# staple/spark-agd

Measured on NVIDIA H100. Metric: AGD examples/sec (rows x applySmooth passes / s), logistic 10M x 1024 dense fp32, higher is better.
Workload: dtype f64

## Files before the change

### spark-agd_b200/csrc/k1_tc.cu

```cuda
#include <cuda.h>
#include <cuda_bf16.h>
#include <cuda_runtime.h>
#include <stdint.h>

#include "agd_common.cuh"
#include "k1_device.cuh"

namespace agd {

namespace {

constexpr int kKR = 16;
constexpr int kRegsConsumer = 64, kRegsAux = 56, kRegsMma = 168;
constexpr int kBlockBytes = kKR * 128;
constexpr int kBBytes = 1024;
constexpr int kScaleOff = 768;

__device__ __forceinline__ uint32_t smem_u32(const void *p) { return (uint32_t)__cvta_generic_to_shared(p); }
__device__ __forceinline__ void mbar_init(uint32_t bar, uint32_t count) {
  asm volatile("mbarrier.init.shared::cta.b64 [%0], %1;" ::"r"(bar), "r"(count));
}
__device__ __forceinline__ void mbar_expect_tx(uint32_t bar, uint32_t bytes) {
  asm volatile("mbarrier.arrive.expect_tx.shared::cta.b64 _, [%0], %1;" ::"r"(bar), "r"(bytes) : "memory");
}
__device__ __forceinline__ void mbar_arrive(uint32_t bar) {
  asm volatile("mbarrier.arrive.shared::cta.b64 _, [%0];" ::"r"(bar) : "memory");
}
__device__ __forceinline__ void mbar_wait(uint32_t bar, uint32_t parity) {
  asm volatile(
      "{\n\t.reg .pred p;\n\t"
      "WAIT_LOOP:\n\t"
      "mbarrier.try_wait.parity.shared::cta.b64 p, [%0], %1;\n\t"
      "@p bra WAIT_DONE;\n\t"
      "bra WAIT_LOOP;\n\t"
      "WAIT_DONE:\n\t}" ::"r"(bar),
      "r"(parity)
      : "memory");
}
__device__ __forceinline__ void named_arrive(int id, int count) {
  asm volatile("bar.arrive %0, %1;" ::"r"(id), "r"(count) : "memory");
}
__device__ __forceinline__ void named_sync(int id, int count) {
  asm volatile("bar.sync %0, %1;" ::"r"(id), "r"(count) : "memory");
}
__device__ __forceinline__ void tma_bulk_g2s(uint32_t dst, const void *src, uint32_t bytes, uint32_t bar) {
  asm volatile("cp.async.bulk.shared::cluster.global.mbarrier::complete_tx::bytes [%0], [%1], %2, [%3];" ::"r"(dst),
               "l"(src), "r"(bytes), "r"(bar)
               : "memory");
}
__device__ __forceinline__ void tma_tile_2d(uint32_t dst, const CUtensorMap *map, int c0, int c1, uint32_t bar) {
  asm volatile("cp.async.bulk.tensor.2d.shared::cluster.global.mbarrier::complete_tx::bytes [%0], [%1, {%2, %3}], [%4];" ::"r"(dst),
               "l"(map), "r"(c0), "r"(c1), "r"(bar)
               : "memory");
}
__device__ __forceinline__ void tma_tile_3d(uint32_t dst, const CUtensorMap *map, int c0, int c1, int c2, uint32_t bar) {
  asm volatile("cp.async.bulk.tensor.3d.shared::cluster.global.mbarrier::complete_tx::bytes [%0], [%1, {%2, %3, %4}], [%5];" ::"r"(dst),
               "l"(map), "r"(c0), "r"(c1), "r"(c2), "r"(bar)
               : "memory");
}
__device__ __forceinline__ uint64_t gmma_desc(uint32_t addr, uint32_t lbo, uint32_t sbo, uint64_t layout) {
  return (uint64_t)((addr & 0x3FFFF) >> 4) | ((uint64_t)(lbo >> 4) << 16) | ((uint64_t)(sbo >> 4) << 32) | (layout << 62);
}
__device__ __forceinline__ void wgmma_fence() { asm volatile("wgmma.fence.sync.aligned;" ::: "memory"); }
__device__ __forceinline__ void wgmma_commit() { asm volatile("wgmma.commit_group.sync.aligned;" ::: "memory"); }
template <int N>
__device__ __forceinline__ void wgmma_wait() { asm volatile("wgmma.wait_group.sync.aligned %0;" ::"n"(N) : "memory"); }
template <int N>
__device__ __forceinline__ void wgmma_bf16(float (&d)[N / 2], uint64_t adesc, uint64_t bdesc);
template <>
__device__ __forceinline__ void wgmma_bf16<16>(float (&d)[8], uint64_t adesc, uint64_t bdesc) {
  asm volatile("{ .reg .pred p; setp.ne.b32 p, 0, 0;\n\t"
               "wgmma.mma_async.sync.aligned.m64n16k16.f32.bf16.bf16 {%0,%1,%2,%3,%4,%5,%6,%7}, %8, %9, p, 1, 1, 1, 0; }"
               : "+f"(d[0]), "+f"(d[1]), "+f"(d[2]), "+f"(d[3]), "+f"(d[4]), "+f"(d[5]), "+f"(d[6]), "+f"(d[7])
               : "l"(adesc), "l"(bdesc)
               : "memory");
}
template <>
__device__ __forceinline__ void wgmma_bf16<24>(float (&d)[12], uint64_t adesc, uint64_t bdesc) {
  asm volatile("{ .reg .pred p; setp.ne.b32 p, 0, 0;\n\t"
               "wgmma.mma_async.sync.aligned.m64n24k16.f32.bf16.bf16 {%0,%1,%2,%3,%4,%5,%6,%7,%8,%9,%10,%11}, %12, %13, p, 1, 1, 1, 0; }"
               : "+f"(d[0]), "+f"(d[1]), "+f"(d[2]), "+f"(d[3]), "+f"(d[4]), "+f"(d[5]), "+f"(d[6]), "+f"(d[7]),
                 "+f"(d[8]), "+f"(d[9]), "+f"(d[10]), "+f"(d[11])
               : "l"(adesc), "l"(bdesc)
               : "memory");
}

template <int N, bool TWO>
__device__ __forceinline__ void mma_accumulate(const float (&e)[2][N / 2], int hb, int hs, const double (&sc)[2], double &g,
                                               double *g2) {
  float v[6];
#pragma unroll
  for (int t = 0; t < (TWO ? 6 : 3); ++t) {
    const int i = t == 0 ? 0 : t == 1 ? 1 : t == 2 ? 4 : t == 3 ? 5 : t == 4 ? 8 : 9;
    const float x0 = hs ? e[0][i + 2] : e[0][i], x1 = hs ? e[1][i + 2] : e[1][i];
    v[t] = hb ? x1 : x0;
  }
  g += (((double)v[0] + (double)v[1]) + (double)v[2]) * sc[0];
  if (TWO) *g2 += (((double)v[3] + (double)v[4]) + (double)v[5]) * sc[1];
}
__device__ __forceinline__ double pow2i(int k) { return __longlong_as_double((long long)(k + 1023) << 52); }
__device__ __forceinline__ void mma_release(uint32_t empty_bar, int lane) {
  __syncwarp();
  if (lane == 0) mbar_arrive(empty_bar);
}

struct TcLayout {
  uint32_t ring_off, w_off, b2_off, partial_off, bars_off, g2_off, total;
};
__host__ __device__ inline TcLayout tc_layout(int ring_groups, int group_bytes, int d, bool two_gradient) {
  TcLayout L;
  L.ring_off = 0;
  L.w_off = (uint32_t)ring_groups * group_bytes;
  L.b2_off = L.w_off + (uint32_t)d * 8;
  L.partial_off = L.b2_off + 2 * kBBytes;
  L.bars_off = L.partial_off + 2 * kKR * 16 * 8;
  L.g2_off = L.bars_off + (2 * (uint32_t)ring_groups + 8) * 8;
  L.total = L.g2_off + (two_gradient ? (uint32_t)d * 8 : 0u);
  return L;
}

struct TcArgs {
  const double *labels;
  const double *w;
  const double *w2;
  double *slabs;
  long long rows;
  int d, kind, slab_stride;
  unsigned long long sample_seed, sample_thresh;
  long long row_base;
  const RowFilter *filt;
  const uint32_t *view_bits;
  int gb;
  int ngt;
  int ring_groups;
  int one_copy;
  int diag;
};

__host__ __device__ constexpr int tc_consumers(int rpt) { return rpt == 4 ? 256 : 512; }
__device__ __forceinline__ unsigned long long ffma2(unsigned long long a, unsigned long long b, unsigned long long c) {
  const float x = __fmaf_rn(__uint_as_float((uint32_t)a), __uint_as_float((uint32_t)b), __uint_as_float((uint32_t)c));
  const float y = __fmaf_rn(__uint_as_float((uint32_t)(a >> 32)), __uint_as_float((uint32_t)(b >> 32)),
                            __uint_as_float((uint32_t)(c >> 32)));
  return ((unsigned long long)__float_as_uint(y) << 32) | __float_as_uint(x);
}
__device__ __forceinline__ unsigned long long pack2(uint32_t lo, uint32_t hi) {
  unsigned long long d;
  asm("mov.b64 %0, {%1, %2};" : "=l"(d) : "r"(lo), "r"(hi));
  return d;
}

template <int RPT, bool F32, int DUAL, bool VIEW, bool BIAS>
__global__ void __launch_bounds__(tc_consumers(RPT) + 256, 1)
k1_tc_kernel(const __grid_constant__ CUtensorMap tmap, const __grid_constant__ CUtensorMap tmap3, const TcArgs a,
             const long long ntiles) {
  constexpr int kConsumers = tc_consumers(RPT);
  constexpr int kThreads = kConsumers + 256;
  constexpr int kN = DUAL == 2 ? 24 : 16;
  constexpr int kCW = kConsumers / 32;
  constexpr bool kRepartition = RPT != 4;
  extern __shared__ __align__(1024) unsigned char smem[];
  const int group_bytes = a.gb * kBlockBytes;
  const TcLayout L = tc_layout(a.ring_groups, group_bytes, a.d, DUAL == 2);
  double *w_s = reinterpret_cast<double *>(smem + L.w_off);
  unsigned char *b2 = smem + L.b2_off;
  double *partial = reinterpret_cast<double *>(smem + L.partial_off);
  const uint32_t bars = smem_u32(smem + L.bars_off);
  const int RG = a.ring_groups;
  const uint32_t wbar = bars + 16u * RG, b2_full = wbar + 8, b2_empty = b2_full + 16;
  const int tid = threadIdx.x, warp = tid >> 5, lane = tid & 31;
  const long long my_tiles = (ntiles - blockIdx.x + gridDim.x - 1) / gridDim.x;
  const int npairs = a.d / 128;
  double *slab = a.slabs + (size_t)blockIdx.x * a.slab_stride;

  if (tid == 0) {
    for (int g = 0; g < RG; ++g) {
      mbar_init(bars + 8u * g, 1);
      mbar_init(bars + 8u * (RG + g), 4);
    }
    mbar_init(wbar, 1);
    mbar_init(b2_full, 1); mbar_init(b2_full + 8, 1);
    mbar_init(b2_empty, 4); mbar_init(b2_empty + 8, 4);
    asm volatile("fence.mbarrier_init.release.cluster;" ::: "memory");
  }
  for (int i = tid; i < 2 * kBBytes / 4; i += kThreads) reinterpret_cast<uint32_t *>(b2)[i] = 0u;
  asm volatile("fence.proxy.async.shared::cta;" ::: "memory");
  __syncthreads();

  if (warp >= kCW && warp < kCW + 4) {
   if (kRepartition) asm volatile("setmaxnreg.dec.sync.aligned.u32 %0;" ::"n"(kRegsAux));
   if (warp == kCW) {
    if (lane == 0) {
      mbar_expect_tx(wbar, (uint32_t)a.d * 8u);
      tma_bulk_g2s(smem_u32(w_s), a.w, (uint32_t)a.d * 8u, wbar);
      int slot = -1;
      uint32_t epar = 0;
      bool wrapped = false;
      for (long long k = 0; k < my_tiles; ++k) {
        const long long row0 = (blockIdx.x + k * (long long)gridDim.x) * kKR;
        for (int gi = 0; gi < a.ngt; ++gi) {
          if (++slot == RG) { slot = 0; if (wrapped) epar ^= 1u; wrapped = true; }
          if (wrapped) mbar_wait(bars + 8u * (RG + slot), epar);
          const uint32_t full = bars + 8u * slot;
          mbar_expect_tx(full, (uint32_t)group_bytes);
          if (a.one_copy) {
            tma_tile_3d(smem_u32(smem + (size_t)slot * group_bytes), &tmap3, 0, (int)row0, gi * a.gb, full);
          } else {
            for (int b = 0; b < a.gb; ++b)
              tma_tile_2d(smem_u32(smem + (size_t)slot * group_bytes + b * kBlockBytes), &tmap, (gi * a.gb + b) * 64, (int)row0, full);
          }
        }
      }
    }
   } else if (warp == kCW + 2) {
    double lossacc = 0.0, cntacc = 0.0, multacc = 0.0;
    double ynext = 0.0;
    const int srow = lane & 15;
    const bool second = DUAL && lane >= kKR;
    if (lane < kKR || DUAL) {
      const long long r = (long long)blockIdx.x * kKR + srow;
      if (r < a.rows) ynext = a.labels[r];
    }
    const double *partial2 = partial + 2 * kKR * 2;
    for (long long k = 0; k < my_tiles; ++k) {
      const int bb = (int)(k & 1);
      const long long tile = blockIdx.x + k * (long long)gridDim.x;
      const long long left = a.rows - tile * kKR;
      const int rv = left < kKR ? (int)left : kKR;
      const double ylab = ynext;
      if (lane < kKR || DUAL) {
        const long long r = (tile + gridDim.x) * kKR + srow;
        if (r < a.rows) ynext = a.labels[r];
      }
      named_sync(1 + bb, kConsumers + 32);
      double mult = 0.0;
      bool nonfinite = false;
      if (lane < kKR || second) {
        double m;
        if (RPT) {
          const double *pp = second ? partial2 : partial;
          m = pp[(bb * kKR + srow) * 2] + pp[(bb * kKR + srow) * 2 + 1];
        } else {
          const double *pp = partial + (bb * kKR + lane) * 16;
          m = (((pp[0] + pp[1]) + (pp[2] + pp[3])) + ((pp[4] + pp[5]) + (pp[6] + pp[7]))) +
              (((pp[8] + pp[9]) + (pp[10] + pp[11])) + ((pp[12] + pp[13]) + (pp[14] + pp[15])));
        }
        if (BIAS) m += ld_volatile_f64(second ? a.w2 + a.d : a.w + a.d);
        nonfinite = (lane < kKR || DUAL == 2) && srow < rv && !isfinite(m);
        double mu, loss;
        loss_eval(a.kind, m, ylab, mu, loss);
        if (srow < rv && (!VIEW || ((a.view_bits[(tile * kKR + srow) >> 5] >> ((tile * kKR + srow) & 31)) & 1u) != 0u) &&
            row_selected(a.sample_seed, a.sample_thresh, a.row_base + tile * kKR + srow)) {
          mult = mu; lossacc += loss; cntacc += 1.0;
          if (BIAS) multacc += mu;
        }
      }
      named_arrive(3 + bb, kConsumers + 32);
      const uint32_t hw = (uint32_t)__double2hiint(mult) & 0x7fffffffu;
      const uint32_t hwf = hw | (nonfinite ? 0x80000000u : 0u);
      uint32_t top = __reduce_max_sync(0xffffffffu, lane < kKR ? hwf : 0u), top2 = 0u;
      if (DUAL == 2) top2 = __reduce_max_sync(0xffffffffu, lane < kKR ? 0u : hwf);
      if ((top | top2) >> 31) {
        top = __reduce_max_sync(0xffffffffu, lane < kKR ? hw : 0u);
        if (DUAL == 2) top2 = __reduce_max_sync(0xffffffffu, lane < kKR ? 0u : hw);
        const uint32_t fl = __ballot_sync(0xffffffffu, nonfinite && mult == 0.0);
        const uint32_t zero_rows = DUAL == 2 ? (fl & (fl >> 16) & 0xffffu) : fl;
        const int slot0 = (int)((k * a.ngt) % RG);
#pragma unroll 1
        for (uint32_t rows = zero_rows; rows; rows &= rows - 1u) {
          const int zr = __ffs(rows) - 1;
          int sl = slot0;
#pragma unroll 1
          for (int gi = 0; gi < a.ngt; ++gi) {
#pragma unroll 1
            for (int c = lane; c < a.gb * 8; c += 32)
              *reinterpret_cast<uint4 *>(smem + sl * group_bytes + (c >> 3) * kBlockBytes + zr * 128 + (c & 7) * 16) =
                  make_uint4(0u, 0u, 0u, 0u);
            if (++sl == RG) sl = 0;
          }
        }
      }
      uint32_t E = top >> 20;
      if (DUAL == 2 && second) E = top2 >> 20;
      const int s = E == 0x7ffu ? 0 : E == 0u ? -1022 : E == 0x7feu ? 1023 : (int)E - 1022;
      const int ns = -s;
      const double ms = (mult * pow2i(ns >> 1)) * pow2i(ns - (ns >> 1));
      if (k >= 2) mbar_wait(b2_empty + 8u * bb, (uint32_t)(((k >> 1) - 1) & 1));
      if (srow == 0 && (lane < kKR || (DUAL == 2 && second))) {
        reinterpret_cast<double *>(b2 + bb * kBBytes + kScaleOff)[second ? 1 : 0] = pow2i(s);
      }
      if (lane < kKR || (DUAL == 2 && second)) {
        const __nv_bfloat16 hi = __double2bfloat16(ms);
        const double r1 = ms - (double)__bfloat162float(hi);
        const __nv_bfloat16 mid = __double2bfloat16(r1);
        const double r2 = r1 - (double)__bfloat162float(mid);
        const __nv_bfloat16 lo = __double2bfloat16(r2);
        const int n0 = second ? 9 : 0, n1 = second ? 16 : 1, n2 = second ? 17 : 8;
        unsigned char *base = b2 + bb * kBBytes + (srow / 8) * 128 + (srow % 8) * 2;
#pragma unroll
        for (int t = 0; t < 4; ++t) {
          const int c0 = n0 + 2 * t, c1 = n1 + 2 * t, c2 = n2 + 2 * t;
          *reinterpret_cast<__nv_bfloat16 *>(base + (c0 / 8) * 256 + (c0 % 8) * 16) = hi;
          *reinterpret_cast<__nv_bfloat16 *>(base + (c1 / 8) * 256 + (c1 % 8) * 16) = mid;
          *reinterpret_cast<__nv_bfloat16 *>(base + (c2 / 8) * 256 + (c2 % 8) * 16) = lo;
        }
      }
      asm volatile("fence.proxy.async.shared::cta;" ::: "memory");
      __syncwarp();
      if (lane == 0) mbar_arrive(b2_full + 8u * bb);
    }
    for (int off = DUAL ? 8 : 16; off >= 1; off >>= 1) {
      lossacc += __shfl_xor_sync(0xffffffffu, lossacc, off);
      cntacc += __shfl_xor_sync(0xffffffffu, cntacc, off);
      if (BIAS) multacc += __shfl_xor_sync(0xffffffffu, multacc, off);
    }
    const int DB = a.d + (BIAS ? 1 : 0);
    if (lane == 0) {
      if (BIAS) slab[a.d] = multacc;
      slab[DB] = lossacc; slab[DB + 1] = cntacc; if (!DUAL) { slab[DB + 2] = 0.0; slab[DB + 3] = 0.0; }
    }
    if (DUAL && lane == kKR) {
      slab[DB + 2] = lossacc; slab[DB + 3] = cntacc;
      if (DUAL == 2) {
        double *slab2 = slab + DB + 4;
        if (BIAS) slab2[a.d] = multacc;
        slab2[DB] = lossacc; slab2[DB + 1] = cntacc; slab2[DB + 2] = 0.0; slab2[DB + 3] = 0.0;
      }
    }
   }
  } else if (warp >= kCW + 4) {
    if (kRepartition) asm volatile("setmaxnreg.inc.sync.aligned.u32 %0;" ::"n"(kRegsMma));
    const int mw = warp - (kCW + 4);
    const int q = lane >> 2, j = lane & 3;
    const int hb = j >> 1, hs = j & 1;
    const int fo = 64 * hb + 16 * mw + q + 8 * hs;
    double gacc[32];
#pragma unroll
    for (int p = 0; p < 32; ++p) gacc[p] = 0.0;
    double *g2 = reinterpret_cast<double *>(smem + L.g2_off);
    if (DUAL == 2)
      for (int p = 0; p < npairs; ++p) g2[128 * p + fo] = 0.0;
    const int hp = a.gb / 2;
    int slot = -1;
    uint32_t par = 1;
    float acc[2][kN / 2];
    for (long long k = 0; k < my_tiles; ++k) {
      const int bb = (int)(k & 1);
      mbar_wait(b2_full + 8u * bb, (uint32_t)((k >> 1) & 1));
      const uint64_t bdesc = gmma_desc(smem_u32(b2 + bb * kBBytes), 128, 256, 0);
      const double *scs = reinterpret_cast<const double *>(b2 + bb * kBBytes + kScaleOff);
      const double sc[2] = {scs[0], DUAL == 2 ? scs[1] : 1.0};
#pragma unroll
      for (int p = 0; p < 32; ++p) {
        if (p < npairs) {
          const int pg = p % hp;
          if (pg == 0) {
            if (++slot == RG) slot = 0;
            if (slot == 0) par ^= 1u;
            mbar_wait(bars + 8u * slot, par);
          }
          const uint32_t a0 = smem_u32(smem + (size_t)slot * group_bytes + (2 * pg) * kBlockBytes);
          wgmma_fence();
          if (a.diag != 101) {
            wgmma_bf16<kN>(acc[0], gmma_desc(a0, kBlockBytes, 1024, 1), bdesc);
            wgmma_bf16<kN>(acc[1], gmma_desc(a0 + kBlockBytes, kBlockBytes, 1024, 1), bdesc);
          }
          wgmma_commit();
          wgmma_wait<0>();
          mma_accumulate<kN, DUAL == 2>(acc, hb, hs, sc, gacc[p], g2 + 128 * p + fo);
          if (pg == hp - 1) mma_release(bars + 8u * (RG + slot), lane);
        }
      }
      __syncwarp();
      if (lane == 0) mbar_arrive(b2_empty + 8u * bb);
    }
#pragma unroll
    for (int p = 0; p < 32; ++p)
      if (p < npairs) {
        slab[128 * p + fo] = gacc[p];
        if (DUAL == 2) slab[a.d + (BIAS ? 1 : 0) + 4 + 128 * p + fo] = g2[128 * p + fo];
      }
  } else {
    if (kRepartition) asm volatile("setmaxnreg.dec.sync.aligned.u32 %0;" ::"n"(kRegsConsumer));
    if constexpr (RPT == 0) {
      const int r = lane & 15, hsel = lane >> 4;
      mbar_wait(wbar, 0);
      int slot = -1;
      uint32_t par = 1;
      const int npairs = a.gb * 4;
      uint32_t x_off[2];
      int w_off[2];
      bool act[2];
#pragma unroll
      for (int j = 0; j < 2; ++j) {
        const int c = 2 * (warp + 16 * j) + hsel;
        act[j] = warp + 16 * j < npairs;
        x_off[j] = (uint32_t)((c >> 3) * kBlockBytes + r * 128 + (((c & 7) ^ (r & 7)) << 4));
        w_off[j] = c * 8;
      }
      for (long long k = 0; k < my_tiles; ++k) {
        const int bb = (int)(k & 1);
        double pa[2] = {0.0, 0.0}, pb[2] = {0.0, 0.0};
        const double *wp = w_s;
        for (int gi = 0; gi < a.ngt; ++gi) {
          if (++slot == RG) slot = 0;
          if (slot == 0) par ^= 1u;
          mbar_wait(bars + 8u * slot, par);
          if (a.diag != 100) {
            const unsigned char *gbase = smem + (uint32_t)slot * (uint32_t)group_bytes;
#pragma unroll
            for (int j = 0; j < 2; ++j) {
              if (act[j]) {
                const uint4 xr = *reinterpret_cast<const uint4 *>(gbase + x_off[j]);
                const double2 *wv = reinterpret_cast<const double2 *>(wp + w_off[j]);
#pragma unroll
                for (int q = 0; q < 4; ++q) {
                  const double2 wq = wv[q];
                  const uint32_t xw = q == 0 ? xr.x : q == 1 ? xr.y : q == 2 ? xr.z : xr.w;
                  pa[j] = fma((double)__uint_as_float(xw << 16), wq.x, pa[j]);
                  pb[j] = fma((double)__uint_as_float(xw & 0xffff0000u), wq.y, pb[j]);
                }
              }
            }
          }
          wp += a.gb * 64;
        }
        double p = (pa[0] + pb[0]) + (pa[1] + pb[1]);
        p += __shfl_xor_sync(0xffffffffu, p, 16);
        if (k >= 2) named_sync(3 + bb, kConsumers + 32);
        if (lane < 16) partial[(bb * kKR + r) * 16 + warp] = p;
        named_arrive(1 + bb, kConsumers + 32);
      }
    } else {
    constexpr int kSlots = kKR / (RPT ? RPT : 1);
    const int rq = tid >> 6;
    const int vv = tid & 63;
    mbar_wait(wbar, 0);
    int slot = -1;
    uint32_t par = 1;
    const int blk = vv >> 3, ch = vv & 7;
    const bool active = vv < a.gb * 8;
    uint32_t x_off[RPT];
#pragma unroll
    for (int j = 0; j < RPT; ++j) {
      const int row = rq + j * kSlots;
      x_off[j] = (uint32_t)(blk * kBlockBytes + row * 128 + ((ch ^ (row & 7)) << 4));
    }
    if constexpr (F32) {
      const int nchunks = a.d / 8;
      float4 lo4[2], hi4[2], lo4b[2], hi4b[2];
#pragma unroll
      for (int i = 0; i < 2; ++i) {
        const int c = tid + i * kConsumers;
        if (c < nchunks) {
          const double *src = w_s + (size_t)c * 8;
          lo4[i] = make_float4((float)src[0], (float)src[1], (float)src[2], (float)src[3]);
          hi4[i] = make_float4((float)src[4], (float)src[5], (float)src[6], (float)src[7]);
          if (DUAL) {
            const double *s2 = a.w2 + (size_t)c * 8;
            lo4b[i] = make_float4((float)s2[0], (float)s2[1], (float)s2[2], (float)s2[3]);
            hi4b[i] = make_float4((float)s2[4], (float)s2[5], (float)s2[6], (float)s2[7]);
          }
        }
      }
      named_sync(5, kConsumers);
      float4 *plane0 = reinterpret_cast<float4 *>(w_s), *plane1 = plane0 + nchunks;
      float4 *plane0b = plane1 + nchunks, *plane1b = plane0b + nchunks;
#pragma unroll
      for (int i = 0; i < 2; ++i) {
        const int c = tid + i * kConsumers;
        if (c < nchunks) {
          plane0[c] = lo4[i]; plane1[c] = hi4[i];
          if (DUAL) { plane0b[c] = lo4b[i]; plane1b[c] = hi4b[i]; }
        }
      }
      named_sync(5, kConsumers);
      double *partial2 = partial + 2 * kKR * 2;
      for (long long k = 0; k < my_tiles; ++k) {
        const int bb = (int)(k & 1);
        double pd[RPT], pd2[RPT];
        unsigned long long acc[RPT], acc2[RPT];
#pragma unroll
        for (int j = 0; j < RPT; ++j) { pd[j] = 0.0; acc[j] = 0ull; pd2[j] = 0.0; acc2[j] = 0ull; }
        const ulonglong2 *wp0 = reinterpret_cast<const ulonglong2 *>(plane0) + vv;
        const ulonglong2 *wp1 = reinterpret_cast<const ulonglong2 *>(plane1) + vv;
        const ulonglong2 *wq0 = reinterpret_cast<const ulonglong2 *>(plane0b) + vv;
        const ulonglong2 *wq1 = reinterpret_cast<const ulonglong2 *>(plane1b) + vv;
        for (int gi = 0; gi < a.ngt; ++gi) {
          if (++slot == RG) slot = 0;
          if (slot == 0) par ^= 1u;
          mbar_wait(bars + 8u * slot, par);
          if (active && a.diag != 100) {
            const unsigned char *gbase = smem + (uint32_t)slot * (uint32_t)group_bytes;
            uint4 xr[RPT];
#pragma unroll
            for (int j = 0; j < RPT; ++j) xr[j] = *reinterpret_cast<const uint4 *>(gbase + x_off[j]);
            const ulonglong2 wa = *wp0, wb = *wp1;
            ulonglong2 va = wa, vb = wb;
            if (DUAL) { va = *wq0; vb = *wq1; }
#pragma unroll
            for (int j = 0; j < RPT; ++j) {
              const unsigned long long x0 = pack2(xr[j].x << 16, xr[j].x & 0xffff0000u), x1 = pack2(xr[j].y << 16, xr[j].y & 0xffff0000u),
                                       x2 = pack2(xr[j].z << 16, xr[j].z & 0xffff0000u), x3 = pack2(xr[j].w << 16, xr[j].w & 0xffff0000u);
              acc[j] = ffma2(x0, wa.x, acc[j]);
              acc[j] = ffma2(x1, wa.y, acc[j]);
              acc[j] = ffma2(x2, wb.x, acc[j]);
              acc[j] = ffma2(x3, wb.y, acc[j]);
              if (DUAL) {
                acc2[j] = ffma2(x0, va.x, acc2[j]);
                acc2[j] = ffma2(x1, va.y, acc2[j]);
                acc2[j] = ffma2(x2, vb.x, acc2[j]);
                acc2[j] = ffma2(x3, vb.y, acc2[j]);
              }
            }
          }
          wp0 += a.gb * 8;
          wp1 += a.gb * 8;
          wq0 += a.gb * 8;
          wq1 += a.gb * 8;
          if ((gi & 1) || gi + 1 == a.ngt) {
#pragma unroll
            for (int j = 0; j < RPT; ++j) {
              pd[j] += (double)(__uint_as_float((uint32_t)acc[j]) + __uint_as_float((uint32_t)(acc[j] >> 32)));
              acc[j] = 0ull;
              if (DUAL) {
                pd2[j] += (double)(__uint_as_float((uint32_t)acc2[j]) + __uint_as_float((uint32_t)(acc2[j] >> 32)));
                acc2[j] = 0ull;
              }
            }
          }
        }
        const double tot = warp_rows_reduce<RPT>(pd, lane);
        double tot2 = 0.0;
        if (DUAL) tot2 = warp_rows_reduce<RPT>(pd2, lane);
        if (k >= 2) named_sync(3 + bb, kConsumers + 32);
        if ((lane & (32 / RPT - 1)) == 0) {
          partial[(bb * kKR + rq + kSlots * (lane / (32 / RPT))) * 2 + (warp & 1)] = tot;
          if (DUAL) partial2[(bb * kKR + rq + kSlots * (lane / (32 / RPT))) * 2 + (warp & 1)] = tot2;
        }
        named_arrive(1 + bb, kConsumers + 32);
      }
    } else {
    for (int c = tid; c < a.d / 8; c += kConsumers) {
      const int f = (c >> 1) & 3;
      if (f) {
        double2 *blk = reinterpret_cast<double2 *>(w_s + (size_t)c * 8);
        const double2 t0 = blk[0], t1 = blk[1], t2 = blk[2], t3 = blk[3];
        const double2 v[4] = {t0, t1, t2, t3};
        blk[0 ^ f] = v[0]; blk[1 ^ f] = v[1]; blk[2 ^ f] = v[2]; blk[3 ^ f] = v[3];
      }
    }
    named_sync(5, kConsumers);
    const int sw = (lane >> 1) & 3;
    for (long long k = 0; k < my_tiles; ++k) {
      const int bb = (int)(k & 1);
      double pa[RPT], pb[RPT];
#pragma unroll
      for (int j = 0; j < RPT; ++j) { pa[j] = 0.0; pb[j] = 0.0; }
      const double *wp = w_s + (blk * 64 + ch * 8);
      for (int gi = 0; gi < a.ngt; ++gi) {
        if (++slot == RG) slot = 0;
        if (slot == 0) par ^= 1u;
        mbar_wait(bars + 8u * slot, par);
        if (active && a.diag != 100) {
          const unsigned char *gbase = smem + (uint32_t)slot * (uint32_t)group_bytes;
          uint4 xr[RPT];
#pragma unroll
          for (int j = 0; j < RPT; ++j) xr[j] = *reinterpret_cast<const uint4 *>(gbase + x_off[j]);
#pragma unroll
          for (int q = 0; q < 4; ++q) {
            const double2 wq = *reinterpret_cast<const double2 *>(wp + 2 * (q ^ sw));
#pragma unroll
            for (int j = 0; j < RPT; ++j) {
              const uint32_t xw = q == 0 ? xr[j].x : q == 1 ? xr[j].y : q == 2 ? xr[j].z : xr[j].w;
              pa[j] = fma((double)__uint_as_float(xw << 16), wq.x, pa[j]);
              pb[j] = fma((double)__uint_as_float(xw & 0xffff0000u), wq.y, pb[j]);
            }
          }
        }
        wp += a.gb * 64;
      }
      double p[RPT];
#pragma unroll
      for (int j = 0; j < RPT; ++j) p[j] = pa[j] + pb[j];
      const double tot = warp_rows_reduce<RPT>(p, lane);
      if (k >= 2) named_sync(3 + bb, kConsumers + 32);
      if ((lane & (32 / RPT - 1)) == 0) partial[(bb * kKR + rq + kSlots * (lane / (32 / RPT))) * 2 + (warp & 1)] = tot;
      named_arrive(1 + bb, kConsumers + 32);
    }
    }
    }
  }
}

template <int SITE, typename K>
cudaError_t set_smem_once(K kern, int bytes) {
  static int cur[64] = {0};
  int dev = 0;
  cudaError_t e = cudaGetDevice(&dev);
  if (e != cudaSuccess) return e;
  if (dev >= 0 && dev < 64 && cur[dev] == bytes) return cudaSuccess;
  e = cudaFuncSetAttribute(kern, cudaFuncAttributeMaxDynamicSharedMemorySize, bytes);
  if (e == cudaSuccess && dev >= 0 && dev < 64) cur[dev] = bytes;
  return e;
}

template <bool VIEW, bool BIAS>
cudaError_t tc_launch_forms(const K1Args &a, const CUtensorMap &tmap, const CUtensorMap &tmap3, const TcArgs &t, long long grid,
                            int smem_bytes, long long ntiles, cudaStream_t st) {
  cudaError_t e;
  if (a.tune_rows == 1) {
    e = set_smem_once<1 + 8 * VIEW + 16 * BIAS>(k1_tc_kernel<0, false, 0, VIEW, BIAS>, smem_bytes);
    if (e != cudaSuccess) return e;
    k1_tc_kernel<0, false, 0, VIEW, BIAS><<<(unsigned)grid, 768, smem_bytes, st>>>(tmap, tmap3, t, ntiles);
  } else if (a.tune_rows == 4) {
    e = set_smem_once<2 + 8 * VIEW + 16 * BIAS>(k1_tc_kernel<4, false, 0, VIEW, BIAS>, smem_bytes);
    if (e != cudaSuccess) return e;
    k1_tc_kernel<4, false, 0, VIEW, BIAS><<<(unsigned)grid, 512, smem_bytes, st>>>(tmap, tmap3, t, ntiles);
  } else if (a.tc_margins_f64) {
    e = set_smem_once<3 + 8 * VIEW + 16 * BIAS>(k1_tc_kernel<2, false, 0, VIEW, BIAS>, smem_bytes);
    if (e != cudaSuccess) return e;
    k1_tc_kernel<2, false, 0, VIEW, BIAS><<<(unsigned)grid, 768, smem_bytes, st>>>(tmap, tmap3, t, ntiles);
  } else if (a.w2 && a.dual_full) {
    e = set_smem_once<6 + 8 * VIEW + 16 * BIAS>(k1_tc_kernel<2, true, 2, VIEW, BIAS>, smem_bytes);
    if (e != cudaSuccess) return e;
    k1_tc_kernel<2, true, 2, VIEW, BIAS><<<(unsigned)grid, 768, smem_bytes, st>>>(tmap, tmap3, t, ntiles);
  } else if (a.w2) {
    e = set_smem_once<4 + 8 * VIEW + 16 * BIAS>(k1_tc_kernel<2, true, 1, VIEW, BIAS>, smem_bytes);
    if (e != cudaSuccess) return e;
    k1_tc_kernel<2, true, 1, VIEW, BIAS><<<(unsigned)grid, 768, smem_bytes, st>>>(tmap, tmap3, t, ntiles);
  } else {
    e = set_smem_once<5 + 8 * VIEW + 16 * BIAS>(k1_tc_kernel<2, true, 0, VIEW, BIAS>, smem_bytes);
    if (e != cudaSuccess) return e;
    k1_tc_kernel<2, true, 0, VIEW, BIAS><<<(unsigned)grid, 768, smem_bytes, st>>>(tmap, tmap3, t, ntiles);
  }
  return cudaGetLastError();
}

typedef CUresult (*EncodeTiledFn)(CUtensorMap *, CUtensorMapDataType, cuuint32_t, void *, const cuuint64_t *, const cuuint64_t *,
                                  const cuuint32_t *, const cuuint32_t *, CUtensorMapInterleave, CUtensorMapSwizzle,
                                  CUtensorMapL2promotion, CUtensorMapFloatOOBfill);

}

int k1_tc_supported(int32_t d, int elem_bytes) { return elem_bytes == 2 && d >= 128 && d <= 4096 && d % 128 == 0; }

cudaError_t k1_tc_launch(const K1Args &a, int bias, int sm_count, int *blocks_out, cudaStream_t st) {
  if (!k1_tc_supported(a.d, 2)) return cudaErrorInvalidValue;
  if (a.rows <= 0) { *blocks_out = 0; return cudaSuccess; }
  static EncodeTiledFn encode = nullptr;
  if (!encode) {
    void *fn = nullptr;
    cudaDriverEntryPointQueryResult qres;
    cudaError_t e = cudaGetDriverEntryPoint("cuTensorMapEncodeTiled", &fn, cudaEnableDefault, &qres);
    if (e != cudaSuccess || !fn) return e != cudaSuccess ? e : cudaErrorUnknown;
    encode = (EncodeTiledFn)fn;
  }
  CUtensorMap tmap;
  const cuuint64_t gdim[2] = {(cuuint64_t)a.d, (cuuint64_t)a.rows};
  const cuuint64_t gstr[1] = {(cuuint64_t)a.d * 2};
  const cuuint32_t box[2] = {64, (cuuint32_t)kKR};
  const cuuint32_t estr[2] = {1, 1};
  if (encode(&tmap, CU_TENSOR_MAP_DATA_TYPE_BFLOAT16, 2, const_cast<void *>(a.X), gdim, gstr, box, estr,
             CU_TENSOR_MAP_INTERLEAVE_NONE, CU_TENSOR_MAP_SWIZZLE_128B, CU_TENSOR_MAP_L2_PROMOTION_L2_256B,
             CU_TENSOR_MAP_FLOAT_OOB_FILL_NONE) != CUDA_SUCCESS)
    return cudaErrorInvalidValue;
  const int nblk = a.d / 64;
  int gb = 8;
  while (nblk % gb) gb -= 2;
  CUtensorMap tmap3;
  {
    const cuuint64_t gdim3[3] = {64, (cuuint64_t)a.rows, (cuuint64_t)nblk};
    const cuuint64_t gstr3[2] = {(cuuint64_t)a.d * 2, 128};
    const cuuint32_t box3[3] = {64, (cuuint32_t)kKR, (cuuint32_t)gb};
    const cuuint32_t estr3[3] = {1, 1, 1};
    if (encode(&tmap3, CU_TENSOR_MAP_DATA_TYPE_BFLOAT16, 3, const_cast<void *>(a.X), gdim3, gstr3, box3, estr3,
               CU_TENSOR_MAP_INTERLEAVE_NONE, CU_TENSOR_MAP_SWIZZLE_128B, CU_TENSOR_MAP_L2_PROMOTION_L2_256B,
               CU_TENSOR_MAP_FLOAT_OOB_FILL_NONE) != CUDA_SUCCESS)
      return cudaErrorInvalidValue;
  }
  TcArgs t;
  t.one_copy = a.tune_ctas == 2 ? 0 : 1;
  t.diag = (a.kind == 100 || a.kind == 101) ? a.kind : 0;
  if (a.w2 && (a.tune_rows != 0 || a.tc_margins_f64)) return cudaErrorInvalidValue;
  t.labels = a.labels; t.w = a.w; t.w2 = a.w2; t.slabs = a.slabs; t.rows = a.rows; t.d = a.d; t.kind = a.kind;
  t.slab_stride = a.slab_stride;
  t.sample_seed = a.sample_seed; t.sample_thresh = a.sample_thresh; t.row_base = a.row_base; t.filt = a.filt; t.view_bits = a.view_bits;
  t.gb = gb;
  t.ngt = nblk / gb;
  const int group_bytes = t.gb * kBlockBytes;
  int ring = a.stages > 0 ? a.stages : 16;
  const bool two_gradient = a.w2 && a.dual_full;
  const uint32_t budget = 227u * 1024u - 2048u;
  while (ring > 2 && tc_layout(ring, group_bytes, a.d, two_gradient).total + 1024 > budget) --ring;
  if (ring < t.ngt + 1) ring = t.ngt + 1;
  t.ring_groups = ring;
  const TcLayout L = tc_layout(ring, group_bytes, a.d, two_gradient);
  if (L.total + 1024 > budget) return cudaErrorInvalidValue;
  const long long ntiles = (a.rows + kKR - 1) / kKR;
  long long grid = sm_count;
  if (grid > ntiles) grid = ntiles;
  *blocks_out = (int)grid;
  const int smem_bytes = (int)L.total + 1024;
  if (bias)
    return a.filt ? tc_launch_forms<true, true>(a, tmap, tmap3, t, grid, smem_bytes, ntiles, st)
                  : tc_launch_forms<false, true>(a, tmap, tmap3, t, grid, smem_bytes, ntiles, st);
  return a.filt ? tc_launch_forms<true, false>(a, tmap, tmap3, t, grid, smem_bytes, ntiles, st)
                : tc_launch_forms<false, false>(a, tmap, tmap3, t, grid, smem_bytes, ntiles, st);
}

}
```

Measured before the change: 1.089 billion.

## Issue four wgmma pairs per ring group and drain with staged waits

Adds a QUAD template path, used when the group size is 8, in which consumers issue four wgmma pairs per ring slot into four accumulator sets. Each set is then drained behind its own wgmma_wait<3..0>, instead of fully waiting after every single pair, so MMA latency overlaps with the FP64 accumulation. It also drops the per-CTA zeroing of the B operand buffer. To compensate, the producer writes the lo term into an extra column and the single-gradient accumulate ORs in a fourth fragment, which relies on unused columns staying consistent. The diag 101 mode is now rejected. The extra accumulator sets raise register pressure in the consumer warps.

```diff
diff --git a/spark-agd_b200/csrc/k1_tc.cu b/spark-agd_b200/csrc/k1_tc.cu
--- a/spark-agd_b200/csrc/k1_tc.cu
+++ b/spark-agd_b200/csrc/k1_tc.cu
@@ -90,11 +90,12 @@
                                                double *g2) {
   float v[6];
 #pragma unroll
-  for (int t = 0; t < (TWO ? 6 : 3); ++t) {
+  for (int t = 0; t < (TWO ? 6 : 4); ++t) {
     const int i = t == 0 ? 0 : t == 1 ? 1 : t == 2 ? 4 : t == 3 ? 5 : t == 4 ? 8 : 9;
     const float x0 = hs ? e[0][i + 2] : e[0][i], x1 = hs ? e[1][i + 2] : e[1][i];
     v[t] = hb ? x1 : x0;
   }
+  if (!TWO) v[2] = __uint_as_float(__float_as_uint(v[2]) | __float_as_uint(v[3]));
   g += (((double)v[0] + (double)v[1]) + (double)v[2]) * sc[0];
   if (TWO) *g2 += (((double)v[3] + (double)v[4]) + (double)v[5]) * sc[1];
 }
@@ -150,7 +151,7 @@
   return d;
 }
 
-template <int RPT, bool F32, int DUAL, bool VIEW, bool BIAS>
+template <int RPT, bool F32, int DUAL, bool VIEW, bool BIAS, bool QUAD = false>
 __global__ void __launch_bounds__(tc_consumers(RPT) + 256, 1)
 k1_tc_kernel(const __grid_constant__ CUtensorMap tmap, const __grid_constant__ CUtensorMap tmap3, const TcArgs a,
              const long long ntiles) {
@@ -183,8 +184,6 @@
     mbar_init(b2_empty, 4); mbar_init(b2_empty + 8, 4);
     asm volatile("fence.mbarrier_init.release.cluster;" ::: "memory");
   }
-  for (int i = tid; i < 2 * kBBytes / 4; i += kThreads) reinterpret_cast<uint32_t *>(b2)[i] = 0u;
-  asm volatile("fence.proxy.async.shared::cta;" ::: "memory");
   __syncthreads();
 
   if (warp >= kCW && warp < kCW + 4) {
@@ -303,6 +302,7 @@
           *reinterpret_cast<__nv_bfloat16 *>(base + (c0 / 8) * 256 + (c0 % 8) * 16) = hi;
           *reinterpret_cast<__nv_bfloat16 *>(base + (c1 / 8) * 256 + (c1 % 8) * 16) = mid;
           *reinterpret_cast<__nv_bfloat16 *>(base + (c2 / 8) * 256 + (c2 % 8) * 16) = lo;
+          if (DUAL != 2) *reinterpret_cast<__nv_bfloat16 *>(base + 256 + (c0 % 8 + 1) * 16) = lo;
         }
       }
       asm volatile("fence.proxy.async.shared::cta;" ::: "memory");
@@ -343,32 +343,66 @@
     const int hp = a.gb / 2;
     int slot = -1;
     uint32_t par = 1;
-    float acc[2][kN / 2];
+    auto issue = [&](float (&e)[2][kN / 2], uint32_t a0, uint64_t bdesc) {
+      wgmma_bf16<kN>(e[0], gmma_desc(a0, kBlockBytes, 1024, 1), bdesc);
+      wgmma_bf16<kN>(e[1], gmma_desc(a0 + kBlockBytes, kBlockBytes, 1024, 1), bdesc);
+      wgmma_commit();
+    };
+    constexpr bool kQuad = QUAD;
+    static_assert(!QUAD || (kN == 16 && kRepartition), "four accumulator sets fit the one- and two-point forms only");
+    constexpr int kSets = kQuad ? 4 : 1;
+    auto drain = [&](float (&e)[2][kN / 2], const double (&sc)[2], double &g) {
+#pragma unroll
+      for (int b = 0; b < 2; ++b)
+#pragma unroll
+        for (int i = 0; i < kN / 2; ++i) asm volatile("" : "+f"(e[b][i])::"memory");
+      mma_accumulate<kN, false>(e, hb, hs, sc, g, nullptr);
+    };
+    float acc[kSets][2][kN / 2];
     for (long long k = 0; k < my_tiles; ++k) {
       const int bb = (int)(k & 1);
       mbar_wait(b2_full + 8u * bb, (uint32_t)((k >> 1) & 1));
       const uint64_t bdesc = gmma_desc(smem_u32(b2 + bb * kBBytes), 128, 256, 0);
       const double *scs = reinterpret_cast<const double *>(b2 + bb * kBBytes + kScaleOff);
       const double sc[2] = {scs[0], DUAL == 2 ? scs[1] : 1.0};
-#pragma unroll
-      for (int p = 0; p < 32; ++p) {
-        if (p < npairs) {
-          const int pg = p % hp;
-          if (pg == 0) {
+      if constexpr (kQuad) {
+#pragma unroll
+        for (int p = 0; p < 32; p += 4) {
+          if (p < npairs) {
             if (++slot == RG) slot = 0;
             if (slot == 0) par ^= 1u;
             mbar_wait(bars + 8u * slot, par);
-          }
-          const uint32_t a0 = smem_u32(smem + (size_t)slot * group_bytes + (2 * pg) * kBlockBytes);
-          wgmma_fence();
-          if (a.diag != 101) {
-            wgmma_bf16<kN>(acc[0], gmma_desc(a0, kBlockBytes, 1024, 1), bdesc);
-            wgmma_bf16<kN>(acc[1], gmma_desc(a0 + kBlockBytes, kBlockBytes, 1024, 1), bdesc);
-          }
-          wgmma_commit();
-          wgmma_wait<0>();
-          mma_accumulate<kN, DUAL == 2>(acc, hb, hs, sc, gacc[p], g2 + 128 * p + fo);
-          if (pg == hp - 1) mma_release(bars + 8u * (RG + slot), lane);
+            const uint32_t a0 = smem_u32(smem + (size_t)slot * group_bytes);
+            wgmma_fence();
+#pragma unroll
+            for (int i = 0; i < 4; ++i) issue(acc[i % kSets], a0 + 2 * i * kBlockBytes, bdesc);
+            wgmma_wait<3>();
+            drain(acc[0], sc, gacc[p]);
+            wgmma_wait<2>();
+            drain(acc[1 % kSets], sc, gacc[p + 1]);
+            wgmma_wait<1>();
+            drain(acc[2 % kSets], sc, gacc[p + 2]);
+            wgmma_wait<0>();
+            drain(acc[3 % kSets], sc, gacc[p + 3]);
+            mma_release(bars + 8u * (RG + slot), lane);
+          }
+        }
+      } else {
+#pragma unroll
+        for (int p = 0; p < 32; ++p) {
+          if (p < npairs) {
+            const int pg = p % hp;
+            if (pg == 0) {
+              if (++slot == RG) slot = 0;
+              if (slot == 0) par ^= 1u;
+              mbar_wait(bars + 8u * slot, par);
+            }
+            wgmma_fence();
+            issue(acc[0], smem_u32(smem + (size_t)slot * group_bytes + (2 * pg) * kBlockBytes), bdesc);
+            wgmma_wait<0>();
+            mma_accumulate<kN, DUAL == 2>(acc[0], hb, hs, sc, gacc[p], g2 + 128 * p + fo);
+            if (pg == hp - 1) mma_release(bars + 8u * (RG + slot), lane);
+          }
         }
       }
       __syncwarp();
@@ -603,6 +637,15 @@
   e = cudaFuncSetAttribute(kern, cudaFuncAttributeMaxDynamicSharedMemorySize, bytes);
   if (e == cudaSuccess && dev >= 0 && dev < 64) cur[dev] = bytes;
   return e;
+}
+
+template <int SITE, typename K>
+cudaError_t tc_launch(K kern, const TcArgs &t, long long grid, int smem_bytes, long long ntiles, cudaStream_t st,
+                      const CUtensorMap &tmap, const CUtensorMap &tmap3) {
+  const cudaError_t e = set_smem_once<SITE>(kern, smem_bytes);
+  if (e != cudaSuccess) return e;
+  kern<<<(unsigned)grid, 768, smem_bytes, st>>>(tmap, tmap3, t, ntiles);
+  return cudaGetLastError();
 }
 
 template <bool VIEW, bool BIAS>
@@ -626,13 +669,11 @@
     if (e != cudaSuccess) return e;
     k1_tc_kernel<2, true, 2, VIEW, BIAS><<<(unsigned)grid, 768, smem_bytes, st>>>(tmap, tmap3, t, ntiles);
   } else if (a.w2) {
-    e = set_smem_once<4 + 8 * VIEW + 16 * BIAS>(k1_tc_kernel<2, true, 1, VIEW, BIAS>, smem_bytes);
-    if (e != cudaSuccess) return e;
-    k1_tc_kernel<2, true, 1, VIEW, BIAS><<<(unsigned)grid, 768, smem_bytes, st>>>(tmap, tmap3, t, ntiles);
+    if (t.gb == 8) return tc_launch<4 + 8 * VIEW + 16 * BIAS>(k1_tc_kernel<2, true, 1, VIEW, BIAS, true>, t, grid, smem_bytes, ntiles, st, tmap, tmap3);
+    return tc_launch<4 + 8 * VIEW + 16 * BIAS>(k1_tc_kernel<2, true, 1, VIEW, BIAS>, t, grid, smem_bytes, ntiles, st, tmap, tmap3);
   } else {
-    e = set_smem_once<5 + 8 * VIEW + 16 * BIAS>(k1_tc_kernel<2, true, 0, VIEW, BIAS>, smem_bytes);
-    if (e != cudaSuccess) return e;
-    k1_tc_kernel<2, true, 0, VIEW, BIAS><<<(unsigned)grid, 768, smem_bytes, st>>>(tmap, tmap3, t, ntiles);
+    if (t.gb == 8) return tc_launch<5 + 8 * VIEW + 16 * BIAS>(k1_tc_kernel<2, true, 0, VIEW, BIAS, true>, t, grid, smem_bytes, ntiles, st, tmap, tmap3);
+    return tc_launch<5 + 8 * VIEW + 16 * BIAS>(k1_tc_kernel<2, true, 0, VIEW, BIAS>, t, grid, smem_bytes, ntiles, st, tmap, tmap3);
   }
   return cudaGetLastError();
 }
@@ -681,7 +722,8 @@
   }
   TcArgs t;
   t.one_copy = a.tune_ctas == 2 ? 0 : 1;
-  t.diag = (a.kind == 100 || a.kind == 101) ? a.kind : 0;
+  if (a.kind == 101) return cudaErrorInvalidValue;
+  t.diag = a.kind == 100 ? a.kind : 0;
   if (a.w2 && (a.tune_rows != 0 || a.tc_margins_f64)) return cudaErrorInvalidValue;
   t.labels = a.labels; t.w = a.w; t.w2 = a.w2; t.slabs = a.slabs; t.rows = a.rows; t.d = a.d; t.kind = a.kind;
   t.slab_stride = a.slab_stride;
```

Result: no change. 1.090 billion (median of 6 runs) (+0.0%).
